# USDA-ARS-GBRU/itsxpress

Hardware: AMD Instinct MI355X
Metric: reads/sec trimmed (ITS2, stand-in taxon Tracheophyta for Fungi) (higher is better)
Workload: dtype u8+f32

## Files before the change

### itsxpress_amd/csrc/engine.hip

```cpp
#include <algorithm>
#include <chrono>
#include <cmath>
#include <cstdio>
#include <cstring>
#include <functional>
#include <map>
#include <memory>
#include <numeric>
#include <atomic>
#include <condition_variable>
#include <mutex>
#include <string_view>
#include <thread>
#include <unordered_map>
#include "detmath.h"
#include "engine.h"
#include "k_api.h"
#include "cluster_multi.h"
#include "fastq_io.h"
#include "iupac.h"
#include "writers.h"

namespace itsx {
void launch_region_offsets(int64_t npairs, const PairRec *pairs, const int32_t *pref, const int64_t *seg_pair_start,
// ... 4766 lines not shown
  return ITSX_OK;
}

int itsx_debug_read_hashes(itsx_ctx *ctx, uint64_t *fwd, uint64_t *rc)
{
  CTXCHK(ctx && fwd && rc);
  HIPCHK(hipSetDevice(ctx->device));
  DBuf<uint64_t> hf, hr;
  HIPCHK(hf.alloc((size_t)ctx->N + 1)); HIPCHK(hr.alloc((size_t)ctx->N + 1));
  if (ctx->N > 0) {
    launch_hash_reads(ctx->rd, 0, 1, hf.p, hr.p, ctx->st);
    HIPCHK(hipMemcpyAsync(fwd, hf.p, (size_t)ctx->N * 8, hipMemcpyDeviceToHost, ctx->st));
    HIPCHK(hipMemcpyAsync(rc, hr.p, (size_t)ctx->N * 8, hipMemcpyDeviceToHost, ctx->st));
  }
  HIPCHK(hipStreamSynchronize(ctx->st));
  return ITSX_OK;
}

int itsx_debug_packed_read(const itsx_ctx *ctx, int64_t i, uint32_t *words, int32_t *nwords, uint32_t *exc, int32_t *nexc)
{
  CTXCHK(ctx && i >= 0 && i < ctx->N && nwords && nexc);
  HIPCHK(hipSetDevice(ctx->device));
  int64_t eo[2] = {0, 0};
  HIPCHK(hipMemcpy(eo, ctx->d_excoff.p + i, sizeof(eo), hipMemcpyDeviceToHost));
  const int32_t nw = (int32_t)(ctx->h_woff[i + 1] - ctx->h_woff[i]), ne = (int32_t)(eo[1] - eo[0]);
  if (words) HIPCHK(hipMemcpy(words, ctx->d_words.p + ctx->h_woff[i], (size_t)nw * 4, hipMemcpyDeviceToHost));
  if (exc && ne) HIPCHK(hipMemcpy(exc, ctx->d_exc.p + eo[0], (size_t)ne * 4, hipMemcpyDeviceToHost));
  *nwords = nw; *nexc = ne;
  return ITSX_OK;
}

int itsx_debug_calibrate(itsx_ctx *ctx, int pattern, double gbytes, int iters, int64_t *bytes_per_launch, double *ms_per_launch)
{
  CTXCHK(ctx && pattern >= 0 && pattern <= 3 && gbytes > 0 && iters >= 1);
  HIPCHK(hipSetDevice(ctx->device));
  const int64_t nwaves = 256 * 32;
  const int64_t row_floats = pattern == 3 ? 4 * 64 : 6 * 64;
  const int64_t R = std::max<int64_t>(1, (int64_t)(gbytes * 1e9) / (nwaves * row_floats * 4));
  DBuf<float> slab, out;
  HIPCHK(slab.alloc((size_t)(nwaves * R * row_floats), true)); HIPCHK(out.alloc((size_t)nwaves * 64));
  HIPCHK(hipMemsetAsync(slab.p, 0, (size_t)(nwaves * R * row_floats) * 4, ctx->st));
  StageTimer tm(ctx->st);
  for (int i = 0; i < iters; i++) launch_calib(pattern, slab.p, nwaves, R, out.p, ctx->st);
  const float ms = tm.stop();
  HIPCHK(hipGetLastError());
  const int64_t touched = pattern == 1 ? 5 * 64 * 4 : row_floats * 4;
  if (bytes_per_launch) *bytes_per_launch = nwaves * R * touched;
  if (ms_per_launch) *ms_per_launch = ms / iters;
  return ITSX_OK;
}

int itsx_debug_issue(itsx_ctx *ctx, int op, int waves_per_simd, int iters, double *cycles_per_instr, double *ms)
{
  CTXCHK(ctx && op >= 0 && op <= 11 && waves_per_simd >= 1 && waves_per_simd <= 8 && (waves_per_simd <= 4 || waves_per_simd % 2 == 0) && iters >= 1);
  HIPCHK(hipSetDevice(ctx->device));
  int ncu = 256;
  { hipDeviceProp_t pr; if (hipGetDeviceProperties(&pr, ctx->device) == hipSuccess) ncu = pr.multiProcessorCount; }
  const int nw = ncu * 4 * waves_per_simd;
  DBuf<unsigned long long> ticks; DBuf<float> sink;
  HIPCHK(ticks.alloc((size_t)nw)); HIPCHK(sink.alloc(1024));
  HIPCHK(hipMemsetAsync(sink.p, 0, 1024 * sizeof(float), ctx->st));
  launch_issue(op, waves_per_simd, 16, ncu, ticks.p, sink.p, ctx->st);
  StageTimer tm(ctx->st);
  launch_issue(op, waves_per_simd, iters, ncu, ticks.p, sink.p, ctx->st);
  const float t = tm.stop();
  HIPCHK(hipGetLastError());
  std::vector<unsigned long long> h((size_t)nw);
  HIPCHK(hipMemcpy(h.data(), ticks.p, h.size() * sizeof(unsigned long long), hipMemcpyDeviceToHost));
  std::sort(h.begin(), h.end());
  if (cycles_per_instr) *cycles_per_instr = (double)h[h.size() / 2] / (64.0 * (double)iters);
  if (ms) *ms = t;
  return ITSX_OK;
}

int itsx_debug_detmath(itsx_ctx *ctx, const double *x, int64_t n, double *out_log, double *out_exp)
{
  CTXCHK(ctx && x && out_log && out_exp && n >= 0);
  HIPCHK(hipSetDevice(ctx->device));
  DBuf<double> dx, dl, de;
  HIPCHK(dx.alloc((size_t)n + 1)); HIPCHK(dl.alloc((size_t)n + 1)); HIPCHK(de.alloc((size_t)n + 1));
  if (n > 0) {
    HIPCHK(hipMemcpyAsync(dx.p, x, (size_t)n * 8, hipMemcpyHostToDevice, ctx->st));
    launch_detmath(dx.p, n, dl.p, de.p, ctx->st);
    HIPCHK(hipMemcpyAsync(out_log, dl.p, (size_t)n * 8, hipMemcpyDeviceToHost, ctx->st));
    HIPCHK(hipMemcpyAsync(out_exp, de.p, (size_t)n * 8, hipMemcpyDeviceToHost, ctx->st));
  }
  HIPCHK(hipStreamSynchronize(ctx->st));
  return ITSX_OK;
}

int itsx_debug_dust(itsx_ctx *ctx, uint8_t *masked)
{
  CTXCHK(ctx && masked);
  HIPCHK(hipSetDevice(ctx->device));
  const int64_t n = ctx->N;
  if (n == 0) return ITSX_OK;
  DBuf<uint32_t> dm;
  HIPCHK(dm.alloc((size_t)ctx->h_woff[n] + 1));
  launch_dust(ctx->rd, dm.p, ctx->st);
  std::vector<uint32_t> h((size_t)ctx->h_woff[n] + 1);
  HIPCHK(hipMemcpyAsync(h.data(), dm.p, h.size() * 4, hipMemcpyDeviceToHost, ctx->st));
  HIPCHK(hipStreamSynchronize(ctx->st));
  HIPCHK(hipGetLastError());
  int64_t o = 0;
  for (int64_t r = 0; r < n; r++)
    for (int p = 0; p < ctx->h_len[r]; p++) masked[o++] = (uint8_t)((h[(size_t)ctx->h_woff[r] + (p >> 5)] >> (p & 31)) & 1u);
  return ITSX_OK;
// ... 19 lines not shown
```

### itsxpress_amd/csrc/k_msv.hip

```cpp
#include <algorithm>
#include <cstdlib>
#include "engine.h"
#include "k_api.h"

namespace itsx {

constexpr int MSV_WT = 16;
typedef short s2 __attribute__((ext_vector_type(2)));
__device__ __forceinline__ s2 as_s2(uint32_t u) { return __builtin_bit_cast(s2, u); }
__device__ __forceinline__ uint32_t as_u(s2 v) { return __builtin_bit_cast(uint32_t, v); }
__device__ __forceinline__ int uni(int v) { return __builtin_amdgcn_readfirstlane(v); }

template <bool SHARE>
__global__ void __launch_bounds__(256, 6) k_msv(MsvArgs a)
{
  __shared__ __attribute__((aligned(16))) uint32_t tab[2][16 * MSV_TW];
  extern __shared__ uint32_t wst[];
  const bool whole = a.wtl > MSV_WT;
  const int s = a.k0 + blockIdx.x * 256 + threadIdx.x;
  const bool valid = s < a.k1;
  int L = 0, nexc = 0, tjb = 0, Lt = 0;
  const uint32_t *wp = a.rd.words;
  const uint32_t *ep = a.rd.exc;
  const int row0 = SHARE ? (a.sl.depth << a.sl.logB) : 0;
  if (valid) {
    const int r = a.seed_read[a.sorted_uniq[s]];
    L = a.rd.len[r];
    wp = a.rd.words + a.rd.woff[r];
    const int64_t eo = a.rd.excoff[r];
    nexc = (int)(a.rd.excoff[r + 1] - eo);
    ep = a.rd.exc + eo;
    Lt = L < a.Lcap ? L : a.Lcap - 1;
    tjb = a.tjb[Lt];
  }
  if (whole) {
    const int nw = (L + 15) >> 4;
    for (int j = 0; j < a.wtl; j++) wst[j * 256 + threadIdx.x] = (j < nw) ? wp[j] : 0u;
  }
  int myend = L, jlev = -1; int64_t jnode = 0;
  if constexpr (SHARE) {
    if (valid && a.sl.endrow) { myend = a.sl.endrow[s]; jlev = a.sl.jlev[s]; jnode = (int64_t)a.sl.jsrc[s] - a.sl.gnode_base; }
  }
  int Lw = valid ? myend : 0;
  for (int d = 32; d >= 1; d >>= 1) { const int o = __shfl_xor(Lw, d, 64); Lw = o > Lw ? o : Lw; }
  Lw = uni(Lw);
  const int Ppad = a.G * 64;
  const int p0 = a.pfirst + blockIdx.y * a.PB;
  const int np = a.plast;
  int p1 = p0 + a.PB; if (p1 > np) p1 = np;
  const int base = 190;
  for (int pj = p0; pj < p1; pj++) {
    const int p = a.plist ? uni(a.plist[pj]) : pj;
    uint32_t *tb = tab[(pj - p0) & 1];
    for (int i = threadIdx.x; i < 16 * MSV_TW; i += 256) tb[i] = a.etab[(size_t)p * 16 * MSV_TW + i];
    __syncthreads();
    const int bias = uni(a.pbias[p]), tec = uni(a.ptec[p]), tbm = uni(a.ptbm[p]);
    const int tjbm = tjb + tbm;
    int bm0 = base - tjbm; bm0 = bm0 < 0 ? 0 : bm0;
    int xJ = 0, xB = bm0, xEmax = 0;
    uint32_t dp[MSV_REGS];
#pragma unroll
    for (int i = 0; i < MSV_REGS; i++) dp[i] = 0;
    if constexpr (SHARE) {
      if (valid && a.sl.depth > 0) {
        const int64_t src_node = (int64_t)a.sl.src[s] - a.sl.node_base;
        const uint4 *src = (const uint4 *)a.sl.slots + (src_node * a.sl.Pb + (pj - a.pfirst)) * MSV_STATE_Q;
#pragma unroll
        for (int q = 0; q < 6; q++) {
          const uint4 v = src[q];
          dp[4 * q] = v.x; dp[4 * q + 1] = v.y; dp[4 * q + 2] = v.z; if (4 * q + 3 < MSV_REGS) dp[4 * q + 3] = v.w;
        }
        const uint4 v = src[6];
        xJ = (int)v.x; xB = (int)v.y; xEmax = (int)v.z;
      }
    }
    int ei = 0;
    int next_exc = nexc > 0 ? (int)(ep[0] >> 4) : 0x7fffffff;
    uint32_t w = 0;
    const int lend = myend;
    int jxJ = -1, jem = 0;
    for (int pos = row0; pos <= Lw; pos++) {
      const int sh = (pos & 15) * 2;
      if (sh == 0) {
        if constexpr (SHARE) {
          if ((pos & ((1 << a.sl.logB) - 1)) == 0 && valid) {
            const int d = pos >> a.sl.logB;
            const unsigned long long m = a.sl.mask[s];
            if (pos > row0 && pos < L && d < 64 && ((m >> d) & 1ull)) {
              const int64_t node = (int64_t)a.sl.node0[s] + __popcll(m & ((1ull << d) - 1ull)) - a.sl.node_base;
              uint4 *dst = (uint4 *)a.sl.slots + (node * a.sl.Pb + (pj - a.pfirst)) * MSV_STATE_Q;
#pragma unroll
              for (int q = 0; q < 6; q++) dst[q] = make_uint4(dp[4 * q], dp[4 * q + 1], dp[4 * q + 2], (4 * q + 3 < MSV_REGS) ? dp[(4 * q + 3) % MSV_REGS] : 0u);
              dst[6] = make_uint4((uint32_t)xJ, (uint32_t)xB, (uint32_t)xEmax, 0u);
            }
            if (d == jlev) {
              const uint4 *g = (const uint4 *)a.sl.gslots + (jnode * a.sl.Pb + (pj - a.pfirst)) * MSV_STATE_Q;
              s2 mx = as_s2(0x80008000u);
#pragma unroll
              for (int q = 0; q < 6; q++) {
                const uint4 v = g[q];
                mx = __builtin_elementwise_max(mx, __builtin_elementwise_add_sat(as_s2(dp[4 * q]), as_s2(v.x)));
                mx = __builtin_elementwise_max(mx, __builtin_elementwise_add_sat(as_s2(dp[4 * q + 1]), as_s2(v.y)));
                mx = __builtin_elementwise_max(mx, __builtin_elementwise_add_sat(as_s2(dp[4 * q + 2]), as_s2(v.z)));
                if (4 * q + 3 < MSV_REGS) mx = __builtin_elementwise_max(mx, __builtin_elementwise_add_sat(as_s2(dp[4 * q + 3]), as_s2(v.w)));
              }
              const uint4 t = g[6];
              int xf = (int)mx.x > (int)mx.y ? (int)mx.x : (int)mx.y;
              const int c1 = xJ + (int)t.x, c2 = xB + (int)t.y, c3 = (int)t.z;
              xf = xf > c1 ? xf : c1; xf = xf > c2 ? xf : c2; xf = xf > c3 ? xf : c3;
              jxJ = xf; jem = xf + tec;
            }
          }
        }
        if (pos >= Lw) break;
        if (!whole && ((pos & 255) == 0 || pos == row0)) {
          const int w0 = (pos >> 8) << 4, nw = (L + 15) >> 4;
#pragma unroll
          for (int j = 0; j < MSV_WT; j++) wst[j * 256 + threadIdx.x] = (w0 + j < nw) ? wp[w0 + j] : 0u;
        }
        w = wst[(whole ? (pos >> 4) : ((pos >> 4) & (MSV_WT - 1))) * 256 + threadIdx.x];
      }
      if (pos < lend) {
        int code = (int)((w >> sh) & 3u);
        if (pos == next_exc) {
          code = (int)(ep[ei] & 15u);
          ei++;
          next_exc = ei < nexc ? (int)(ep[ei] >> 4) : 0x7fffffff;
        }
        const uint4 *e4 = (const uint4 *)(tb + code * MSV_TW);
        uint32_t e[MSV_TW];
#pragma unroll
        for (int q = 0; q < MSV_TW / 4; q++) { const uint4 v = e4[q]; e[4 * q] = v.x; e[4 * q + 1] = v.y; e[4 * q + 2] = v.z; e[4 * q + 3] = v.w; }
        const s2 xBv = as_s2((uint32_t)xB * 0x10001u);
        const uint32_t wrap = dp[MSV_REGS - 1] << 16;
        s2 xEa = as_s2(0u), xEb = as_s2(0u);
#pragma unroll
        for (int r = MSV_REGS - 1; r >= 0; r--) {
          const uint32_t prev = (r > 0) ? dp[r > 0 ? r - 1 : 0] : wrap;
          const s2 sv = __builtin_elementwise_max(as_s2(prev), xBv) + as_s2(e[r]);
          if (r & 1) xEb = __builtin_elementwise_max(xEb, sv); else xEa = __builtin_elementwise_max(xEa, sv);
          dp[r] = as_u(sv);
        }
        const uint32_t xe2 = as_u(__builtin_elementwise_max(xEa, xEb));
        int xE = (int)(xe2 & 0xffffu);
        const int xEh = (int)(xe2 >> 16);
        xE = xE > xEh ? xE : xEh;
        xEmax = xEmax > xE ? xEmax : xE;
        xE -= tec;
        xJ = xJ > xE ? xJ : xE;
        xB = xJ - tjbm; xB = xB > bm0 ? xB : bm0;
      }
    }
    if (valid) {
      if (jxJ >= 0) { xJ = jxJ; xEmax = xEmax > jem ? xEmax : jem; }
      const int ovf = (xEmax + bias >= 255);
      const int thr = a.thr[(size_t)Lt * Ppad + p];
      const int pass = ovf | (xJ >= thr);
      const int xj = ovf ? 255 : xJ;
      a.res[(size_t)p * a.U + s] = (uint16_t)(pass ? (0x100 | xj) : 0);
    }
  }
}

__global__ void __launch_bounds__(256, 6) k_msv_bwd(MsvArgs a)
{
  __shared__ __attribute__((aligned(16))) uint32_t tab[2][16 * MSV_TW];
  extern __shared__ uint32_t wst[];
  const bool whole = a.wtl > MSV_WT;
  const int s = a.k0 + blockIdx.x * 256 + threadIdx.x;
  const bool valid = s < a.k1;
  int L = 0, tjb = 0, mysteps = 0;
  const uint32_t *wp = a.rd.words;
  if (valid) {
    const int r = a.seed_read[a.sorted_uniq[s]];
    L = a.rd.len[r];
    wp = a.rd.words + a.rd.woff[r];
    const int Lt = L < a.Lcap ? L : a.Lcap - 1;
    tjb = a.tjb[Lt];
    mysteps = a.sl.endrow[s];
  }
  const int nw = (L + 15) >> 4;
  if (whole) for (int j = 0; j < a.wtl; j++) wst[j * 256 + threadIdx.x] = (j < nw) ? wp[j] : 0u;
  int nsteps = mysteps;
  for (int d = 32; d >= 1; d >>= 1) { const int o = __shfl_xor(nsteps, d, 64); nsteps = o > nsteps ? o : nsteps; }
  nsteps = (a.sl.dbg & 32) ? 0 : uni(nsteps);
  const int rd = a.sl.depth, logB = a.sl.logB;
  const int A = (L + (1 << logB) - 1) >> logB;
  const int top = (A - rd) << logB;
  const int p0 = a.pfirst + blockIdx.y * a.PB;
  int p1 = p0 + a.PB; if (p1 > a.plast) p1 = a.plast;
  const int base = 190;
  constexpr int NEG = -16384;
  const unsigned long long m = valid ? a.sl.mask[s] : 0ull;
  for (int pj = p0; pj < p1; pj++) {
    const int p = pj;
    uint32_t *tb = tab[(pj - p0) & 1];
    for (int i = threadIdx.x; i < 16 * MSV_TW; i += 256) tb[i] = a.etab[(size_t)p * 16 * MSV_TW + i];
    __syncthreads();
    const int tec = uni(a.ptec[p]), tbm = uni(a.ptbm[p]);
    const int tjbm = tjb + tbm;
    int bm0 = base - tjbm; bm0 = bm0 < 0 ? 0 : bm0;
    int gJ = 0, gB = NEG, g0 = NEG;
    uint32_t g[MSV_REGS];
#pragma unroll
    for (int i = 0; i < MSV_REGS; i++) g[i] = 0xC000C000u;
    if (valid && rd > 0) {
      const int64_t src_node = (int64_t)a.sl.src[s] - a.sl.node_base;
      const uint4 *src = (const uint4 *)a.sl.slots + (src_node * a.sl.Pb + (pj - a.pfirst)) * MSV_STATE_Q;
// ... 18 lines not shown
        }
      }
      if (step >= nsteps) break;
      const int row = top - step;
      if (row <= L && step < mysteps) {
        const int pos = row - 1;
        if ((pos >> 4) != wi) {
          wi = pos >> 4;
          if (whole) w = wst[wi * 256 + threadIdx.x];
          else w = wp[wi];
        }
        const int code = (int)((w >> ((pos & 15) * 2)) & 3u);
        const uint4 *e4 = (const uint4 *)(tb + code * MSV_TW);
        uint32_t e[MSV_TW];
#pragma unroll
        for (int q = 0; q < MSV_TW / 4; q++) { const uint4 v = e4[q]; e[4 * q] = v.x; e[4 * q + 1] = v.y; e[4 * q + 2] = v.z; e[4 * q + 3] = v.w; }
        int aJ = gB - tjbm; aJ = aJ > gJ ? aJ : gJ;
        const int n0 = gB + bm0; g0 = g0 > n0 ? g0 : n0;
        int aE = aJ - tec; aE = aE > 30000 ? 30000 : aE;
        const s2 aEv = as_s2((uint32_t)(aE & 0xffff) * 0x10001u);
        s2 mxa = as_s2(0xC000C000u), mxb = as_s2(0xC000C000u);
        const s2 W0 = __builtin_elementwise_add_sat(__builtin_elementwise_max(as_s2(g[0]), aEv), as_s2(e[0]));
        mxa = __builtin_elementwise_max(mxa, W0);
#pragma unroll
        for (int r = 1; r < MSV_REGS; r++) {
          const s2 Wr = __builtin_elementwise_add_sat(__builtin_elementwise_max(as_s2(g[r]), aEv), as_s2(e[r]));
          if (r & 1) mxb = __builtin_elementwise_max(mxb, Wr); else mxa = __builtin_elementwise_max(mxa, Wr);
          g[r - 1] = as_u(Wr);
        }
        g[MSV_REGS - 1] = (as_u(W0) >> 16) | 0xC0000000u;
        const uint32_t m2 = as_u(__builtin_elementwise_max(mxa, mxb));
        const int lo = (int)(int16_t)(m2 & 0xffffu), hi = (int)(int16_t)(m2 >> 16);
        gB = lo > hi ? lo : hi;
        gJ = aJ;
      }
    }
  }
}

void launch_msv(const MsvArgs &a0, hipStream_t st, int lds_pad)
{
  MsvArgs a = a0;
  if (a.k1 <= 0) { a.k0 = 0; a.k1 = a.U; }
  if (a.plast <= 0) { a.pfirst = 0; a.plast = a.plist ? a.nlist : a.P; }
  const int np = a.plast - a.pfirst, nk = a.k1 - a.k0;
  if (nk <= 0 || np <= 0) return;
  const dim3 grid((unsigned)((nk + 255) / 256), (unsigned)((np + a.PB - 1) / a.PB));
  static const bool allow_whole = !(sw_get("ITSX_MSV_WHOLE") && atoi(sw_get("ITSX_MSV_WHOLE")) == 0);
  const int need = (a.Lcap - 1 + 15) / 16;
  a.wtl = (allow_whole && need > MSV_WT && need <= 37) ? need : MSV_WT;
  static const bool bwd_whole = sw_get("ITSX_MSV_BWD_WHOLE") && atoi(sw_get("ITSX_MSV_BWD_WHOLE")) != 0;
  if (a.share == 2 && !bwd_whole) a.wtl = MSV_WT;
  const size_t lds = std::max<size_t>((size_t)lds_pad, (a.share == 2 && !bwd_whole) ? 0 : (size_t)a.wtl * 256 * sizeof(uint32_t));
  if (a.share == 2) hipLaunchKernelGGL(k_msv_bwd, grid, dim3(256), lds, st, a);
  else if (a.share) hipLaunchKernelGGL(k_msv<true>, grid, dim3(256), lds, st, a);
  else hipLaunchKernelGGL(k_msv<false>, grid, dim3(256), lds, st, a);
}

__global__ void __launch_bounds__(256) k_pair_count(const uint16_t *__restrict__ res, int32_t U, int32_t nchunks, int32_t *__restrict__ cnt, int32_t *__restrict__ real)
{
  __shared__ int32_t ws[4], wr[4];
  const int p = blockIdx.y, c = blockIdx.x;
  const int64_t base = (int64_t)p * U;
  int32_t n = 0, nr = 0;
  for (int i = threadIdx.x; i < CHUNK; i += 256) {
    const int s = c * CHUNK + i;
    if (s < U) { const int v = res[base + s]; n += (v & 0x300) != 0; nr += (v >> 8) & 1; }
  }
  for (int d = 32; d >= 1; d >>= 1) { n += __shfl_down(n, d, 64); nr += __shfl_down(nr, d, 64); }
  if ((threadIdx.x & 63) == 0) { ws[threadIdx.x >> 6] = n; wr[threadIdx.x >> 6] = nr; }
  __syncthreads();
  if (threadIdx.x == 0) {
    cnt[(int64_t)p * nchunks + c] = ws[0] + ws[1] + ws[2] + ws[3];
    const int32_t r = wr[0] + wr[1] + wr[2] + wr[3];
    if (r) atomicAdd(&real[p], r);
  }
}
__global__ void __launch_bounds__(256) k_chunk_scan(int32_t *__restrict__ cnt, int32_t nchunks, int32_t *__restrict__ total)
{
  __shared__ int32_t ws[4];
  __shared__ int32_t carry;
  int32_t *row = cnt + (int64_t)blockIdx.x * nchunks;
  if (threadIdx.x == 0) carry = 0;
  __syncthreads();
  for (int b = 0; b < nchunks; b += 256) {
    const int i = b + threadIdx.x;
    const int32_t v = i < nchunks ? row[i] : 0;
    int32_t inc = v;
    const int lane = threadIdx.x & 63, wid = threadIdx.x >> 6;
    for (int d = 1; d < 64; d <<= 1) { const int32_t t = __shfl_up(inc, d, 64); if (lane >= d) inc += t; }
    if (lane == 63) ws[wid] = inc;
    __syncthreads();
    int32_t off = carry;
    for (int w = 0; w < wid; w++) off += ws[w];
    if (i < nchunks) row[i] = off + inc - v;
    __syncthreads();
    if (threadIdx.x == 255) carry = off + inc;
    __syncthreads();
  }
  if (threadIdx.x == 0) total[blockIdx.x] = carry;
}
__global__ void __launch_bounds__(256) k_pair_fill(const uint16_t *__restrict__ res, int32_t U, int32_t nchunks, const int32_t *__restrict__ cnt,
                                                   const int64_t *__restrict__ seg_start, const int32_t *__restrict__ ulen,
                                                   PairRec *__restrict__ pairs)
{
  __shared__ int32_t ws[4];
  const int p = blockIdx.y, c = blockIdx.x;
  const int64_t base = (int64_t)p * U;
  const int64_t out0 = seg_start[p] + cnt[(int64_t)p * nchunks + c];
// ... 47 lines not shown
```

### itsxpress_amd/csrc/k_util.hip

```cpp
#include <algorithm>
#include "engine.h"
#include "k_api.h"
#include "detmath.h"

namespace itsx {

constexpr int SCAN_BLOCK = 256;
constexpr int SCAN_ITEMS = 8;
constexpr int SCAN_TILE = SCAN_BLOCK * SCAN_ITEMS;

__global__ void __launch_bounds__(SCAN_BLOCK) k_scan_tiles(const int32_t *__restrict__ in, int32_t *__restrict__ out,
                                                           int64_t n, int32_t *__restrict__ sums)
{
  __shared__ int32_t wsum[SCAN_BLOCK / 64];
  const int64_t base = (int64_t)blockIdx.x * SCAN_TILE + (int64_t)threadIdx.x * SCAN_ITEMS;
  int32_t v[SCAN_ITEMS];
  int32_t tsum = 0;
#pragma unroll
  for (int i = 0; i < SCAN_ITEMS; i++) { v[i] = (base + i < n) ? in[base + i] : 0; tsum += v[i]; }
  const int lane = threadIdx.x & 63, wid = threadIdx.x >> 6;
  int32_t inc = tsum;
#pragma unroll
  for (int d = 1; d < 64; d <<= 1) { const int32_t t = __shfl_up(inc, d, 64); if (lane >= d) inc += t; }
  if (lane == 63) wsum[wid] = inc;
// ... 47 lines not shown
void launch_logf_fast(const float *x, int64_t n, const LogTab *tab, float *out, hipStream_t st)
{
  if (n <= 0) return;
  hipLaunchKernelGGL(k_logf_fast, dim3((unsigned)((n + 255) / 256)), dim3(256), 0, st, x, n, tab, out);
}
void launch_detmath(const double *x, int64_t n, double *ol, double *oe, hipStream_t st)
{
  if (n <= 0) return;
  hipLaunchKernelGGL(k_detmath, dim3((unsigned)((n + 255) / 256)), dim3(256), 0, st, x, n, ol, oe);
}

}

namespace itsx {
__global__ void __launch_bounds__(64) k_calib_read4(const float *__restrict__ slab, int64_t R, int nf, float *__restrict__ out)
{
  const int lane = threadIdx.x;
  const int64_t r0 = (int64_t)blockIdx.x * R;
  float acc = 0.f;
  for (int64_t r = 0; r < R; r++)
    for (int f = 0; f < nf; f++) acc += slab[((r0 + r) * 6 + f) * 64 + lane];
  out[(int64_t)blockIdx.x * 64 + lane] = acc;
}
__global__ void __launch_bounds__(64) k_calib_write4(float *__restrict__ slab, int64_t R, int nf)
{
  const int lane = threadIdx.x;
  const int64_t r0 = (int64_t)blockIdx.x * R;
  for (int64_t r = 0; r < R; r++)
    for (int f = 0; f < nf; f++) slab[((r0 + r) * 6 + f) * 64 + lane] = (float)(r + f);
}
__global__ void __launch_bounds__(64) k_calib_read16(const float4 *__restrict__ slab, int64_t R, float *__restrict__ out)
{
  const int lane = threadIdx.x;
  const int64_t r0 = (int64_t)blockIdx.x * R;
  float acc = 0.f;
  for (int64_t r = 0; r < R; r++) { const float4 v = slab[(r0 + r) * 64 + lane]; acc += v.x + v.y + v.z + v.w; }
  out[(int64_t)blockIdx.x * 64 + lane] = acc;
}
template <int OP>
__device__ __forceinline__ void issue16(float (&x)[32], float a, float b)
{
#pragma unroll
  for (int i = 0; i < 16; i++) {
    if (OP == 0) asm volatile("v_fma_f32 %0, %0, %1, %2" : "+v"(x[i]) : "v"(a), "v"(b));
    else if (OP == 1) asm volatile("v_pk_fma_f32 %0, %0, %1, %1" : "+v"(*(float2 *)&x[2 * i]) : "v"(*(float2 *)&x[0]));
    else if (OP == 2) asm volatile("v_pk_max_i16 %0, %0, %1" : "+v"(x[i]) : "v"(a));
    else if (OP == 3) asm volatile("v_pk_add_u16 %0, %0, %1" : "+v"(x[i]) : "v"(a));
    else if (OP == 4) asm volatile("v_pk_mul_f32 %0, %0, %1" : "+v"(*(float2 *)&x[2 * i]) : "v"(*(float2 *)&x[0]));
    else if (OP == 5) asm volatile("v_pk_add_f32 %0, %0, %1" : "+v"(*(float2 *)&x[2 * i]) : "v"(*(float2 *)&x[0]));
    else if (OP == 6) asm volatile("s_nop 0");
    else if (OP == 7) asm volatile("v_mul_f32 %0, %0, %1" : "+v"(x[i]) : "v"(a));
    else if (OP == 8) asm volatile("v_pk_mov_b32 %0, %1, %1 op_sel:[0,1]" : "=v"(*(float2 *)&x[2 * i]) : "v"(*(float2 *)&x[(2 * i + 2) & 31]));
    else if (OP == 9) asm volatile("v_max_i16 %0, %0, %1" : "+v"(x[i]) : "v"(a));
  }
}
template <int OP>
__device__ __forceinline__ void sload16(float (&x)[32], const float *tab)
{
#pragma unroll
  for (int i = 0; i < 16; i++) {
    asm volatile("s_waitcnt lgkmcnt(0)\n\ts_load_dwordx8 s[36:43], %0, %1\n\ts_load_dwordx8 s[44:51], %0, %2"
                 :: "s"(tab), "n"(i * 64), "n"(i * 64 + 32)
                 : "s36", "s37", "s38", "s39", "s40", "s41", "s42", "s43", "s44", "s45", "s46", "s47", "s48", "s49", "s50", "s51", "memory");
    if (OP == 11) {
#pragma unroll
      for (int k = 0; k < 12; k++) asm volatile("v_pk_fma_f32 %0, %0, %1, %1" : "+v"(*(float2 *)&x[2 * ((i + k) & 15)]) : "v"(*(float2 *)&x[0]));
    }
  }
}
template <int OP>
__global__ void __launch_bounds__(1024) k_issue(int iters, unsigned long long *__restrict__ ticks, float *__restrict__ sink)
{
  float x[32];
#pragma unroll
  for (int i = 0; i < 32; i++) x[i] = 1.0f + 1e-6f * (float)(threadIdx.x + i);
  const float a = 0.999999f, b = 1e-7f;
  __syncthreads();
  const unsigned long long t0 = __builtin_amdgcn_s_memtime();
  if constexpr (OP >= 10) { for (int it = 0; it < iters; it++) { sload16<OP>(x, sink); sload16<OP>(x, sink); sload16<OP>(x, sink); sload16<OP>(x, sink); } }
  else for (int it = 0; it < iters; it++) { issue16<OP>(x, a, b); issue16<OP>(x, a, b); issue16<OP>(x, a, b); issue16<OP>(x, a, b); }
  asm volatile("s_waitcnt lgkmcnt(0)\n\ts_nop 0" ::: "memory");
  const unsigned long long t1 = __builtin_amdgcn_s_memtime();
  float s = 0.f;
#pragma unroll
  for (int i = 0; i < 32; i++) s += x[i];
  if ((threadIdx.x & 63) == 0) ticks[(size_t)blockIdx.x * (blockDim.x >> 6) + (threadIdx.x >> 6)] = t1 - t0;
  if (s == 12345.678f) sink[0] = s;
}
void launch_issue(int op, int waves_per_simd, int iters, int blocks, unsigned long long *ticks, float *sink, hipStream_t st)
{
  const int per_cu = waves_per_simd > 4 ? 2 : 1;
  const dim3 g((unsigned)(blocks * per_cu)), b((unsigned)(256 * waves_per_simd / per_cu));
  const size_t lds = per_cu == 1 ? 96 * 1024 : 0;
  switch (op) {
    case 0: hipLaunchKernelGGL(k_issue<0>, g, b, lds, st, iters, ticks, sink); break;
    case 1: hipLaunchKernelGGL(k_issue<1>, g, b, lds, st, iters, ticks, sink); break;
    case 2: hipLaunchKernelGGL(k_issue<2>, g, b, lds, st, iters, ticks, sink); break;
    case 3: hipLaunchKernelGGL(k_issue<3>, g, b, lds, st, iters, ticks, sink); break;
    case 4: hipLaunchKernelGGL(k_issue<4>, g, b, lds, st, iters, ticks, sink); break;
    case 5: hipLaunchKernelGGL(k_issue<5>, g, b, lds, st, iters, ticks, sink); break;
    case 6: hipLaunchKernelGGL(k_issue<6>, g, b, lds, st, iters, ticks, sink); break;
    case 7: hipLaunchKernelGGL(k_issue<7>, g, b, lds, st, iters, ticks, sink); break;
    case 8: hipLaunchKernelGGL(k_issue<8>, g, b, lds, st, iters, ticks, sink); break;
    case 9: hipLaunchKernelGGL(k_issue<9>, g, b, lds, st, iters, ticks, sink); break;
    case 10: hipLaunchKernelGGL(k_issue<10>, g, b, lds, st, iters, ticks, sink); break;
    default: hipLaunchKernelGGL(k_issue<11>, g, b, lds, st, iters, ticks, sink); break;
  }
}

void launch_calib(int pattern, float *slab, int64_t nwaves, int64_t R, float *out, hipStream_t st)
{
  if (pattern == 0) hipLaunchKernelGGL(k_calib_read4, dim3((unsigned)nwaves), dim3(64), 0, st, slab, R, 6, out);
  else if (pattern == 1) hipLaunchKernelGGL(k_calib_read4, dim3((unsigned)nwaves), dim3(64), 0, st, slab, R, 5, out);
  else if (pattern == 2) hipLaunchKernelGGL(k_calib_write4, dim3((unsigned)nwaves), dim3(64), 0, st, slab, R, 6);
  else hipLaunchKernelGGL(k_calib_read16, dim3((unsigned)nwaves), dim3(64), 0, st, (const float4 *)slab, R, out);
}
}

namespace itsx {
struct __attribute__((packed, aligned(1))) Raw16 { uint32_t a, b, c, d; };
__device__ __forceinline__ bool pack16_plain(const uint8_t *p, uint32_t &w)
{
  const Raw16 v = *(const Raw16 *)p;
  const uint32_t d[4] = {v.a, v.b, v.c, v.d};
  bool plain = true;
  w = 0;
#pragma unroll
  for (int q = 0; q < 4; q++) {
#pragma unroll
    for (int t = 0; t < 4; t++) {
      const uint32_t c = (d[q] >> (8 * t)) & 0xffu, u = c & 0xdfu;
      plain = plain && ((u & 0xe0u) == 0x40u) && (((0x0010008au >> (u & 31u)) & 1u) != 0u);
      const uint32_t x = (c >> 1) & 3u;
      w |= (x ^ (x >> 1)) << (2 * (4 * q + t));
    }
  }
  return plain;
}
constexpr int PACK_RB = 64;
__global__ void __launch_bounds__(256) k_pack_words(const uint8_t *__restrict__ raw, int64_t raw_base, const int64_t *__restrict__ off,
                                                    const int64_t *__restrict__ woff, int64_t r0, int64_t r1, const int8_t *__restrict__ lut,
                                                    uint32_t *__restrict__ words, int32_t *__restrict__ excnt, long long *__restrict__ first_bad)
{
  __shared__ int8_t code[256];
  __shared__ int32_t s_orel[PACK_RB + 1], s_wrel[PACK_RB + 1];
  __shared__ int32_t s_ne[PACK_RB];
  __shared__ int32_t s_bad;
  code[threadIdx.x] = lut[threadIdx.x];
  const int tid = (int)threadIdx.x;
  const int64_t ngroups = (r1 - r0 + PACK_RB - 1) / PACK_RB;
  for (int64_t g = blockIdx.x; g < ngroups; g += gridDim.x) {
    const int64_t first = r0 + g * PACK_RB;
    const int nr = (int)(r1 - first < PACK_RB ? r1 - first : PACK_RB);
    const int64_t o0 = off[first], w0 = woff[first];
    __syncthreads();
    if (tid <= nr) { s_orel[tid] = (int32_t)(off[first + tid] - o0); s_wrel[tid] = (int32_t)(woff[first + tid] - w0); }
    if (tid < PACK_RB) s_ne[tid] = 0;
    if (tid == 0) s_bad = PACK_RB;
    __syncthreads();
// ... 70 lines not shown
```

### itsxpress_amd/csrc/switches.cpp

```cpp
#include "switches.h"
#include <cstdlib>
#include <cstring>

namespace itsx {

static const Switch g_sw[] = {
  {"ITSX_NO_ENSEMBLE", SW_HOOK, "multidomain regions keep their region as one envelope instead of hmmsearch's stochastic-traceback clustering (changes envelopes)"},
  {"ITSX_LAZY_ZUB_SCALE", SW_HOOK, "multiplies the lazy stage's upper bound on domZ: more undecided rows for the completion tests"},
  {"ITSX_LAZY_FORCE_PENDING", SW_HOOK, "treats rows as undecided so that the completion path runs"},
  {"ITSX_LAZY_NO_RERUN", SW_HOOK, "skips the full re-search safety net (leaves undecided rows undecided)"},
  {"ITSX_LAZY_NO_COMPLETE", SW_HOOK, "skips itsx_lazy_complete inside itsx_search_finalize (leaves undecided rows undecided)"},
  {"ITSX_COMPACT_ZMAX", SW_HOOK, "largest domZ the compact / lazy modes call a row 'certain' for (default 1e9); a value below the data's domZ can drop a winner"},
  {"ITSX_COMPACT_DOME_MIN", SW_HOOK, "smallest --domE the compact / lazy modes call a row 'certain' for (default 1e-2)"},
  {"ITSX_PASSA_DBG", SW_HOOK, "pass A diagnostic bits (no rows / no restore / no join): timings only, scores are garbage"},
  {"ITSX_ROWS", SW_MODE, "rows mode when the caller did not call itsx_set_rows_mode: full | compact | lazy (coordinates identical in all three)"},
  {"ITSX_COMPACT_ROWS", SW_MODE, "=1: rows mode compact (older spelling of ITSX_ROWS=compact)"},
  {"ITSX_QMASK", SW_MODE, "=none: vsearch's --qmask none for cluster_size / orient seeds (default dust, as vsearch)"},
  {"ITSX_KEEP_TRACE", SW_MODE, "keeps per-pair filter traces for itsx_get_pairtraces (forces the compact path of a lazy search)"},
  {"ITSX_GZIP_LEVEL", SW_MODE, "deflate level of the trimmed-FASTQ writers (default 6; output bytes differ, records do not)"},
  {"ITSX_TEST_HOOKS", SW_DIAG, "=1: honour the HOOK switches above"},
  {"ITSX_SHARE_CHECK", SW_DIAG, "runs the unshared kernels beside the shared ones and counts differences (itsx_stats.share_mismatch, join_maxdiff)"},
  {"ITSX_LAZY_CHECK_BOUND", SW_DIAG, "compares pass A's scores with HMMER's own Forward arithmetic (itsx_stats.lazy_bound_maxdiff)"},
  {"ITSX_LAZY_HIST", SW_DIAG, "prints the histogram of round-2 candidates per group"},
  {"ITSX_PASSA_DUMP", SW_DIAG, "prints every pass-A launch's waves and wave-rows (scripts/passa_launches.py)"},
  {"ITSX_TRACE_ALLOC", SW_DIAG, "prints every hipMalloc / free with its time"},
  {"ITSX_CL_DEBUG", SW_DIAG, "clustering: prints per-window counters"},
  {"ITSX_MR_DEBUG", SW_DIAG, "ensemble stage: prints per-batch counters"},
  {"ITSX_SHARE", SW_TUNING, "=0: no prefix sharing (round 4's schedule)"},
  {"ITSX_SHARE_TWO", SW_TUNING, "=0: one-sided (prefix-only) sharing for pass A"},
  {"ITSX_MSV_TWO", SW_TUNING, "=0: the MSV filter keeps the one-sided (prefix-only) schedule when pass A shares two-sidedly"},
  {"ITSX_SHARE_B", SW_TUNING, "rows per block of the prefix / suffix trees (default 32)"},
  {"ITSX_SHARE_GB", SW_TUNING, "budget of the saved row states, GB"},
  {"ITSX_SHARE_MIN", SW_TUNING, "smallest shared-row fraction for which the shared schedule is used (default 0.10)"},
  {"ITSX_SHARE_FWD_STREAMS", SW_TUNING, "1 | 2 streams for pass A's batches"},
  {"ITSX_SHARE_MSV_STREAMS", SW_TUNING, "1 | 2 streams for the MSV filter's batches"},
  {"ITSX_NO_CHAINREC", SW_TUNING, "pass A reads a chain's data through the round-5 arrays instead of its 64-byte record (A/B)"},
  {"ITSX_BOUND_FOLD", SW_TUNING, "=0: pass A's plain recurrences instead of the folded ones (also switches two-sided sharing off)"},
  {"ITSX_BOUND_RESCALE_EXP", SW_TUNING, "power of ten at which pass A rescales a row (default 20)"},
  {"ITSX_LAZY_TOPUP", SW_TUNING, "=0: undecided rows go straight to the full count of their profiles (no top-up round); =2: the round also looks for unreported pairs among a profile's weakest (rows settled from above)"},
  {"ITSX_LAZY_EXACT_BOUND", SW_TUNING, "pass A through the HMMER-order Forward kernel (A/B)"},
  {"ITSX_CHUNK_UNIQUES", SW_TUNING, "representatives per search chunk"},
  {"ITSX_MSV_OVERLAP", SW_TUNING, "=0: the next chunk's MSV filter does not run beside the domain stage"},
  {"ITSX_MSV_PAD", SW_TUNING, "dynamic LDS of the overlapped MSV launch (an occupancy cap)"},
  {"ITSX_MSV_WHOLE", SW_TUNING, "=0: MSV stages 16 words at a time even when the whole read fits LDS"},
  {"ITSX_BIAS_OVERLAP", SW_TUNING, "=0: the bias filter does not run on the second stream"},
  {"ITSX_ST2_PRIO", SW_TUNING, "priority of the second stream"},
  {"ITSX_LOAD_PRIORITY", SW_TUNING, "=0: loads do not use the high-priority stream"},
  {"ITSX_SLAB_GB", SW_TUNING, "DP slab budget, GB"},
  {"ITSX_SLAB_ADAPT", SW_TUNING, "=0: the slab budget does not adapt to the job"},
  {"ITSX_DEFER_FREE_GB", SW_TUNING, "device memory kept on the deferred-free list, GB"},
  {"ITSX_MR_LONG_FRAC", SW_TUNING, "ensemble stage: share of regions taken as 'long'"},
  {"ITSX_MR_LONG_LANES", SW_TUNING, "ensemble stage: lanes per long region"},
  {"ITSX_MSV_BWD_WHOLE", SW_TUNING, "=1: the MSV filter's Backward chains copy their whole read to LDS first (A/B arm: same cells)"},
  {"ITSX_LAZY_TOPUP_ALL", SW_TUNING, "=0: a profile whose undecided rows need most of its pairs is left to the full count (itsx_lazy_complete) instead of taking all its unevaluated pairs in the top-up round (same rows)"},
  {"ITSX_MR_WAVES", SW_TUNING, "ensemble stage: waves a batch is spread over (lanes per wave = regions / this, 2 .. 64); 0 = waves of 64 lanes"},
  {"ITSX_MR_ONE_MAX", SW_TUNING, "ensemble stage: a batch of at most this many regions (default 2048) is walked one region per wave with the matrix in LDS; 0 = never"},
  {"ITSX_CL_NOSCORE", SW_TUNING, "clustering: skips the score-only pre-pass (A/B arm; the walk then aligns every candidate: same outcomes)"},
  {"ITSX_CL_NOPRECHECK", SW_TUNING, "clustering: skips the certificate pre-check (A/B arm: same outcomes)"},
  {"ITSX_CL_CAPACITY", SW_TUNING, "clustering: candidate-list capacity"},
  {"ITSX_CL_CCAP", SW_TUNING, "clustering: centroid capacity step"},
  {"ITSX_CL_HEAVY", SW_TUNING, "clustering: heavy-word split on / off"},
  {"ITSX_CL_HEAVY_MIN", SW_TUNING, "clustering: centroids a word needs to count as conserved"},
  {"ITSX_CL_ROWS", SW_TUNING, "clustering: alignment rows per lane"},
  {"ITSX_CL_WINDOW", SW_TUNING, "clustering: queries per speculative window"},
  {"ITSX_PACK_CHUNK", SW_TUNING, "reads per packing launch"},
  {"ITSX_PACK_ECAP", SW_TUNING, "initial capacity of the exception list"},
  {"ITSX_HUGEPAGES", SW_TUNING, "=0: host buffers without MADV_HUGEPAGE"},
  {"ITSX_IO_LIBDEFLATE", SW_TUNING, "=0: zlib instead of libdeflate when both are present"},
  {"ITSX_IO_THREADS", SW_TUNING, "host threads of the FASTQ readers / writers"},
  {"ITSX_IO_BLOCK_KB", SW_TUNING, "deflate unit of the block-parallel writer"},
  {"ITSX_PARALLEL_INFLATE", SW_TUNING, "=0: single-stream inflate"},
  {"ITSX_PINFLATE_CHUNK_KB", SW_TUNING, "chunk of the block-parallel inflater"},
  {"ITSX_PARSE_MIN_MB", SW_TUNING, "smallest text parsed on several threads"},
  {"ITSX_TEXT_CACHE_GB", SW_TUNING, "inflated-text cache, GB"},
  {"ITSX_WRITE_MIN_MB", SW_TUNING, "smallest output written by several threads"},
  {"ITSX_WRITE_UNIT_KB", SW_TUNING, "unit of the streamed writer"},
  {"ITSX_STREAM_RESERVE_MB", SW_TUNING, "streamed loads: first reservation"},
  {"ITSX_STREAM_RESERVE_X", SW_TUNING, "streamed loads: growth factor"},
};
static const int g_nsw = (int)(sizeof(g_sw) / sizeof(g_sw[0]));

const Switch *sw_registry(int *n) { if (n) *n = g_nsw; return g_sw; }

static bool hooks_on() { const char *e = sw_get("ITSX_TEST_HOOKS"); return e && atoi(e) == 1; }

const char *sw_get(const char *name)
{
  const char *v = getenv(name);
  if (!v) return nullptr;
  for (int i = 0; i < g_nsw; i++)
    if (strcmp(g_sw[i].name, name) == 0) return (g_sw[i].kind == SW_HOOK && !hooks_on()) ? nullptr : v;
  return nullptr;
}

std::string sw_report()
{
  std::string out;
// ... 13 lines not shown
```

Before: 4.589 million.

## Use offset-floored saturating DP row in MSV filter to drop per-cell max

Adds a FLOOR template arm to the MSV kernel. Once no lane can still have its J-state below the begin floor, the DP state is rebased relative to xB, and each cell becomes one saturating packed add instead of max+add. The offset is reapplied when states are shared or joined, and dp is shifted only when xB rises in some lane. Overflow detection now derives from xJ rather than a tracked xEmax, and a microbenchmark op for v_pk_add_i16 clamp is added. This risks subtle score or overflow differences and adds code size and register pressure from the duplicated row loop.

Result: faster. 4.663 million (median of 6 runs) (+1.6%).

```diff
diff --git a/itsxpress_amd/csrc/engine.hip b/itsxpress_amd/csrc/engine.hip
--- a/itsxpress_amd/csrc/engine.hip
+++ b/itsxpress_amd/csrc/engine.hip
@@ -4842,7 +4842,7 @@
 
 int itsx_debug_issue(itsx_ctx *ctx, int op, int waves_per_simd, int iters, double *cycles_per_instr, double *ms)
 {
-  CTXCHK(ctx && op >= 0 && op <= 11 && waves_per_simd >= 1 && waves_per_simd <= 8 && (waves_per_simd <= 4 || waves_per_simd % 2 == 0) && iters >= 1);
+  CTXCHK(ctx && op >= 0 && op <= 12 && waves_per_simd >= 1 && waves_per_simd <= 8 && (waves_per_simd <= 4 || waves_per_simd % 2 == 0) && iters >= 1);
   HIPCHK(hipSetDevice(ctx->device));
   int ncu = 256;
   { hipDeviceProp_t pr; if (hipGetDeviceProperties(&pr, ctx->device) == hipSuccess) ncu = pr.multiProcessorCount; }
diff --git a/itsxpress_amd/csrc/k_msv.hip b/itsxpress_amd/csrc/k_msv.hip
--- a/itsxpress_amd/csrc/k_msv.hip
+++ b/itsxpress_amd/csrc/k_msv.hip
@@ -1,5 +1,6 @@
 #include <algorithm>
 #include <cstdlib>
+#include <type_traits>
 #include "engine.h"
 #include "k_api.h"
 
@@ -10,8 +11,9 @@
 __device__ __forceinline__ s2 as_s2(uint32_t u) { return __builtin_bit_cast(s2, u); }
 __device__ __forceinline__ uint32_t as_u(s2 v) { return __builtin_bit_cast(uint32_t, v); }
 __device__ __forceinline__ int uni(int v) { return __builtin_amdgcn_readfirstlane(v); }
-
-template <bool SHARE>
+__device__ __forceinline__ s2 real_off(bool floored, int xB) { return as_s2(floored ? (uint32_t)((xB + 32768) & 0xffff) * 0x10001u : 0u); }
+
+template <bool SHARE, bool FLOOR>
 __global__ void __launch_bounds__(256, 6) k_msv(MsvArgs a)
 {
   __shared__ __attribute__((aligned(16))) uint32_t tab[2][16 * MSV_TW];
@@ -57,7 +59,7 @@
     const int bias = uni(a.pbias[p]), tec = uni(a.ptec[p]), tbm = uni(a.ptbm[p]);
     const int tjbm = tjb + tbm;
     int bm0 = base - tjbm; bm0 = bm0 < 0 ? 0 : bm0;
-    int xJ = 0, xB = bm0, xEmax = 0;
+    int xJ = 0, xB = bm0;
     uint32_t dp[MSV_REGS];
 #pragma unroll
     for (int i = 0; i < MSV_REGS; i++) dp[i] = 0;
@@ -71,15 +73,21 @@
           dp[4 * q] = v.x; dp[4 * q + 1] = v.y; dp[4 * q + 2] = v.z; if (4 * q + 3 < MSV_REGS) dp[4 * q + 3] = v.w;
         }
         const uint4 v = src[6];
-        xJ = (int)v.x; xB = (int)v.y; xEmax = (int)v.z;
+        xJ = (int)v.x; xB = (int)v.y;
       }
     }
     int ei = 0;
     int next_exc = nexc > 0 ? (int)(ep[0] >> 4) : 0x7fffffff;
     uint32_t w = 0;
     const int lend = myend;
-    int jxJ = -1, jem = 0;
-    for (int pos = row0; pos <= Lw; pos++) {
+    int jxJ = -1;
+    int pos = row0;
+    auto rows = [&](auto fast_c) -> bool {
+    constexpr bool FAST = decltype(fast_c)::value;
+    for (; pos <= Lw; pos++) {
+      if constexpr (FLOOR && !FAST) {
+        if (__builtin_amdgcn_ballot_w64(pos < lend && xJ + tec < bm0) == 0ull) return true;
+      }
       const int sh = (pos & 15) * 2;
       if (sh == 0) {
         if constexpr (SHARE) {
@@ -89,30 +97,34 @@
             if (pos > row0 && pos < L && d < 64 && ((m >> d) & 1ull)) {
               const int64_t node = (int64_t)a.sl.node0[s] + __popcll(m & ((1ull << d) - 1ull)) - a.sl.node_base;
               uint4 *dst = (uint4 *)a.sl.slots + (node * a.sl.Pb + (pj - a.pfirst)) * MSV_STATE_Q;
-#pragma unroll
-              for (int q = 0; q < 6; q++) dst[q] = make_uint4(dp[4 * q], dp[4 * q + 1], dp[4 * q + 2], (4 * q + 3 < MSV_REGS) ? dp[(4 * q + 3) % MSV_REGS] : 0u);
-              dst[6] = make_uint4((uint32_t)xJ, (uint32_t)xB, (uint32_t)xEmax, 0u);
+              const s2 ru = real_off(FAST, xB);
+#pragma unroll
+              for (int q = 0; q < 6; q++)
+                dst[q] = make_uint4(as_u(as_s2(dp[4 * q]) + ru), as_u(as_s2(dp[4 * q + 1]) + ru), as_u(as_s2(dp[4 * q + 2]) + ru),
+                                    (4 * q + 3 < MSV_REGS) ? as_u(as_s2(dp[(4 * q + 3) % MSV_REGS]) + ru) : 0u);
+              dst[6] = make_uint4((uint32_t)xJ, (uint32_t)xB, 0u, 0u);
             }
             if (d == jlev) {
               const uint4 *g = (const uint4 *)a.sl.gslots + (jnode * a.sl.Pb + (pj - a.pfirst)) * MSV_STATE_Q;
               s2 mx = as_s2(0x80008000u);
+              const s2 ru = real_off(FAST, xB);
 #pragma unroll
               for (int q = 0; q < 6; q++) {
                 const uint4 v = g[q];
-                mx = __builtin_elementwise_max(mx, __builtin_elementwise_add_sat(as_s2(dp[4 * q]), as_s2(v.x)));
-                mx = __builtin_elementwise_max(mx, __builtin_elementwise_add_sat(as_s2(dp[4 * q + 1]), as_s2(v.y)));
-                mx = __builtin_elementwise_max(mx, __builtin_elementwise_add_sat(as_s2(dp[4 * q + 2]), as_s2(v.z)));
-                if (4 * q + 3 < MSV_REGS) mx = __builtin_elementwise_max(mx, __builtin_elementwise_add_sat(as_s2(dp[4 * q + 3]), as_s2(v.w)));
+                mx = __builtin_elementwise_max(mx, __builtin_elementwise_add_sat(as_s2(dp[4 * q]) + ru, as_s2(v.x)));
+                mx = __builtin_elementwise_max(mx, __builtin_elementwise_add_sat(as_s2(dp[4 * q + 1]) + ru, as_s2(v.y)));
+                mx = __builtin_elementwise_max(mx, __builtin_elementwise_add_sat(as_s2(dp[4 * q + 2]) + ru, as_s2(v.z)));
+                if (4 * q + 3 < MSV_REGS) mx = __builtin_elementwise_max(mx, __builtin_elementwise_add_sat(as_s2(dp[4 * q + 3]) + ru, as_s2(v.w)));
               }
               const uint4 t = g[6];
               int xf = (int)mx.x > (int)mx.y ? (int)mx.x : (int)mx.y;
               const int c1 = xJ + (int)t.x, c2 = xB + (int)t.y, c3 = (int)t.z;
               xf = xf > c1 ? xf : c1; xf = xf > c2 ? xf : c2; xf = xf > c3 ? xf : c3;
-              jxJ = xf; jem = xf + tec;
+              jxJ = xf;
             }
           }
         }
-        if (pos >= Lw) break;
+        if (pos >= Lw) return false;
         if (!whole && ((pos & 255) == 0 || pos == row0)) {
           const int w0 = (pos >> 8) << 4, nw = (L + 15) >> 4;
 #pragma unroll
@@ -131,29 +143,61 @@
         uint32_t e[MSV_TW];
 #pragma unroll
         for (int q = 0; q < MSV_TW / 4; q++) { const uint4 v = e4[q]; e[4 * q] = v.x; e[4 * q + 1] = v.y; e[4 * q + 2] = v.z; e[4 * q + 3] = v.w; }
-        const s2 xBv = as_s2((uint32_t)xB * 0x10001u);
-        const uint32_t wrap = dp[MSV_REGS - 1] << 16;
-        s2 xEa = as_s2(0u), xEb = as_s2(0u);
-#pragma unroll
-        for (int r = MSV_REGS - 1; r >= 0; r--) {
-          const uint32_t prev = (r > 0) ? dp[r > 0 ? r - 1 : 0] : wrap;
-          const s2 sv = __builtin_elementwise_max(as_s2(prev), xBv) + as_s2(e[r]);
-          if (r & 1) xEb = __builtin_elementwise_max(xEb, sv); else xEa = __builtin_elementwise_max(xEa, sv);
-          dp[r] = as_u(sv);
-        }
-        const uint32_t xe2 = as_u(__builtin_elementwise_max(xEa, xEb));
-        int xE = (int)(xe2 & 0xffffu);
-        const int xEh = (int)(xe2 >> 16);
-        xE = xE > xEh ? xE : xEh;
-        xEmax = xEmax > xE ? xEmax : xE;
-        xE -= tec;
-        xJ = xJ > xE ? xJ : xE;
-        xB = xJ - tjbm; xB = xB > bm0 ? xB : bm0;
-      }
+        if constexpr (FAST) {
+          const uint32_t wrap = (dp[MSV_REGS - 1] << 16) | 0x8000u;
+          s2 xEa = as_s2(0x80008000u), xEb = as_s2(0x80008000u);
+#pragma unroll
+          for (int r = MSV_REGS - 1; r >= 0; r--) {
+            const uint32_t prev = (r > 0) ? dp[r > 0 ? r - 1 : 0] : wrap;
+            const s2 sv = __builtin_elementwise_add_sat(as_s2(prev), as_s2(e[r]));
+            if (r & 1) xEb = __builtin_elementwise_max(xEb, sv); else xEa = __builtin_elementwise_max(xEa, sv);
+            dp[r] = as_u(sv);
+          }
+          const uint32_t xe2 = as_u(__builtin_elementwise_max(xEa, xEb));
+          const int xEl = (int)(int16_t)(xe2 & 0xffffu), xEh = (int)xe2 >> 16;
+          const int xE = (xEl > xEh ? xEl : xEh) + xB + (32768 - tec);
+          xJ = xJ > xE ? xJ : xE;
+          int nb = xJ - tjbm; nb = nb > bm0 ? nb : bm0;
+          const int delta = nb - xB;
+          xB = nb;
+          if (__builtin_amdgcn_ballot_w64(delta > 0) != 0ull) {
+            const s2 dv = as_s2((uint32_t)((-delta) & 0xffff) * 0x10001u);
+#pragma unroll
+            for (int i = 0; i < MSV_REGS; i++) dp[i] = as_u(__builtin_elementwise_add_sat(as_s2(dp[i]), dv));
+          }
+        } else {
+          const s2 xBv = as_s2((uint32_t)xB * 0x10001u);
+          const uint32_t wrap = dp[MSV_REGS - 1] << 16;
+          s2 xEa = as_s2(0u), xEb = as_s2(0u);
+#pragma unroll
+          for (int r = MSV_REGS - 1; r >= 0; r--) {
+            const uint32_t prev = (r > 0) ? dp[r > 0 ? r - 1 : 0] : wrap;
+            const s2 sv = __builtin_elementwise_max(as_s2(prev), xBv) + as_s2(e[r]);
+            if (r & 1) xEb = __builtin_elementwise_max(xEb, sv); else xEa = __builtin_elementwise_max(xEa, sv);
+            dp[r] = as_u(sv);
+          }
+          const uint32_t xe2 = as_u(__builtin_elementwise_max(xEa, xEb));
+          int xE = (int)(xe2 & 0xffffu);
+          const int xEh = (int)(xe2 >> 16);
+          xE = xE > xEh ? xE : xEh;
+          xE -= tec;
+          xJ = xJ > xE ? xJ : xE;
+          xB = xJ - tjbm; xB = xB > bm0 ? xB : bm0;
+        }
+      }
+    }
+    return false;
+    };
+    if (rows(std::false_type())) {
+      const s2 xBv = as_s2((uint32_t)xB * 0x10001u);
+      const s2 dn = as_s2((uint32_t)((-(xB + 32768)) & 0xffff) * 0x10001u);
+#pragma unroll
+      for (int i = 0; i < MSV_REGS; i++) dp[i] = as_u(__builtin_elementwise_max(as_s2(dp[i]), xBv) + dn);
+      rows(std::true_type());
     }
     if (valid) {
-      if (jxJ >= 0) { xJ = jxJ; xEmax = xEmax > jem ? xEmax : jem; }
-      const int ovf = (xEmax + bias >= 255);
+      if (jxJ >= 0) xJ = jxJ;
+      const int ovf = (xJ > 0 && xJ + tec + bias >= 255);
       const int thr = a.thr[(size_t)Lt * Ppad + p];
       const int pass = ovf | (xJ >= thr);
       const int xj = ovf ? 255 : xJ;
@@ -278,9 +322,12 @@
   static const bool bwd_whole = sw_get("ITSX_MSV_BWD_WHOLE") && atoi(sw_get("ITSX_MSV_BWD_WHOLE")) != 0;
   if (a.share == 2 && !bwd_whole) a.wtl = MSV_WT;
   const size_t lds = std::max<size_t>((size_t)lds_pad, (a.share == 2 && !bwd_whole) ? 0 : (size_t)a.wtl * 256 * sizeof(uint32_t));
+  const bool floored = !(sw_get("ITSX_MSV_FLOOR") && atoi(sw_get("ITSX_MSV_FLOOR")) == 0);
   if (a.share == 2) hipLaunchKernelGGL(k_msv_bwd, grid, dim3(256), lds, st, a);
-  else if (a.share) hipLaunchKernelGGL(k_msv<true>, grid, dim3(256), lds, st, a);
-  else hipLaunchKernelGGL(k_msv<false>, grid, dim3(256), lds, st, a);
+  else if (a.share && floored) hipLaunchKernelGGL((k_msv<true, true>), grid, dim3(256), lds, st, a);
+  else if (a.share) hipLaunchKernelGGL((k_msv<true, false>), grid, dim3(256), lds, st, a);
+  else if (floored) hipLaunchKernelGGL((k_msv<false, true>), grid, dim3(256), lds, st, a);
+  else hipLaunchKernelGGL((k_msv<false, false>), grid, dim3(256), lds, st, a);
 }
 
 __global__ void __launch_bounds__(256) k_pair_count(const uint16_t *__restrict__ res, int32_t U, int32_t nchunks, int32_t *__restrict__ cnt, int32_t *__restrict__ real)
diff --git a/itsxpress_amd/csrc/k_util.hip b/itsxpress_amd/csrc/k_util.hip
--- a/itsxpress_amd/csrc/k_util.hip
+++ b/itsxpress_amd/csrc/k_util.hip
@@ -123,6 +123,7 @@
     else if (OP == 7) asm volatile("v_mul_f32 %0, %0, %1" : "+v"(x[i]) : "v"(a));
     else if (OP == 8) asm volatile("v_pk_mov_b32 %0, %1, %1 op_sel:[0,1]" : "=v"(*(float2 *)&x[2 * i]) : "v"(*(float2 *)&x[(2 * i + 2) & 31]));
     else if (OP == 9) asm volatile("v_max_i16 %0, %0, %1" : "+v"(x[i]) : "v"(a));
+    else if (OP == 12) asm volatile("v_pk_add_i16 %0, %0, %1 clamp" : "+v"(x[i]) : "v"(a));
   }
 }
 template <int OP>
@@ -148,7 +149,7 @@
   const float a = 0.999999f, b = 1e-7f;
   __syncthreads();
   const unsigned long long t0 = __builtin_amdgcn_s_memtime();
-  if constexpr (OP >= 10) { for (int it = 0; it < iters; it++) { sload16<OP>(x, sink); sload16<OP>(x, sink); sload16<OP>(x, sink); sload16<OP>(x, sink); } }
+  if constexpr (OP == 10 || OP == 11) { for (int it = 0; it < iters; it++) { sload16<OP>(x, sink); sload16<OP>(x, sink); sload16<OP>(x, sink); sload16<OP>(x, sink); } }
   else for (int it = 0; it < iters; it++) { issue16<OP>(x, a, b); issue16<OP>(x, a, b); issue16<OP>(x, a, b); issue16<OP>(x, a, b); }
   asm volatile("s_waitcnt lgkmcnt(0)\n\ts_nop 0" ::: "memory");
   const unsigned long long t1 = __builtin_amdgcn_s_memtime();
@@ -175,7 +176,8 @@
     case 8: hipLaunchKernelGGL(k_issue<8>, g, b, lds, st, iters, ticks, sink); break;
     case 9: hipLaunchKernelGGL(k_issue<9>, g, b, lds, st, iters, ticks, sink); break;
     case 10: hipLaunchKernelGGL(k_issue<10>, g, b, lds, st, iters, ticks, sink); break;
-    default: hipLaunchKernelGGL(k_issue<11>, g, b, lds, st, iters, ticks, sink); break;
+    case 11: hipLaunchKernelGGL(k_issue<11>, g, b, lds, st, iters, ticks, sink); break;
+    default: hipLaunchKernelGGL(k_issue<12>, g, b, lds, st, iters, ticks, sink); break;
   }
 }
 
diff --git a/itsxpress_amd/csrc/switches.cpp b/itsxpress_amd/csrc/switches.cpp
--- a/itsxpress_amd/csrc/switches.cpp
+++ b/itsxpress_amd/csrc/switches.cpp
@@ -43,6 +43,7 @@
   {"ITSX_MSV_OVERLAP", SW_TUNING, "=0: the next chunk's MSV filter does not run beside the domain stage"},
   {"ITSX_MSV_PAD", SW_TUNING, "dynamic LDS of the overlapped MSV launch (an occupancy cap)"},
   {"ITSX_MSV_WHOLE", SW_TUNING, "=0: MSV stages 16 words at a time even when the whole read fits LDS"},
+  {"ITSX_MSV_FLOOR", SW_TUNING, "=0: the MSV filter's plain three-instruction row on every row instead of the floored two-instruction one (A/B arm: same cells; read at every launch)"},
   {"ITSX_BIAS_OVERLAP", SW_TUNING, "=0: the bias filter does not run on the second stream"},
   {"ITSX_ST2_PRIO", SW_TUNING, "priority of the second stream"},
   {"ITSX_LOAD_PRIORITY", SW_TUNING, "=0: loads do not use the high-priority stream"},
```
